# klemens-floege/oneprot

Hardware: AMD Instinct MI355X
Metric: protein-pairs/sec/node (seq+struct-token, L=512, ESM-2-150M) (higher is better)
Workload: dtype bf16; 1 GPU; cfg-2: seq<->struct_token sub-step, facebook/esm2_t30_150M_UR50D / facebook/esm2_t30_150M_UR50D, L=512, 256 pairs/GPU per modality, global batch 256, output_dim 1024, CLIP local_loss+gather_with_grad, L1 0.01, Adam 1e-3, clip 1.0, sequence encoder frozen (reference default), random-init weights; global_batch=256, seq_len=512, parallelism=dp1, frozen_sequence_encoder=True

## Files before the change

include/oneprot_hip.h:

```cpp
#ifndef ONEPROT_HIP_H
#define ONEPROT_HIP_H
#include <stddef.h>
#include <stdint.h>
#ifdef __cplusplus
extern "C" {
#endif

int oneprot_abi_version(void);

int oneprot_esm_embed_fwd(const int64_t* ids, const float* table, float* x, float* row_scale, int B, int L, int d, int vocab,
                          int pad_id, int mask_id, int token_dropout, void* stream);
size_t oneprot_esm_embed_bwd_workspace(int T, int d, int vocab);
int oneprot_esm_embed_bwd(const int64_t* ids, const float* dx, const float* row_scale, float* dtable, void* workspace, int B, int L, int d,
                          int vocab, int pad_id, int mask_id, int token_dropout, int accumulate, void* stream);
int oneprot_bert_embed_fwd(const int64_t* ids, const float* word, const float* pos, const float* type0, const float* gamma, const float* beta,
                           float* x_f32, void* x_bf16, int B, int L, int d, int vocab, float eps, void* stream);

int oneprot_layernorm_fwd(const void* x, int x_is_bf16, const float* gamma, const float* beta, void* y_bf16, float* y_f32, float* mean,
                          float* rstd, int64_t T, int d, float eps, void* stream);
size_t oneprot_layernorm_bwd_workspace(int d);
int oneprot_layernorm_bwd(const void* dy, int dy_mode, const float* wrow, int L, const void* x, int x_is_bf16, const float* gamma,
                          const float* mean, const float* rstd, const float* add_to, float* dx, void* dx_bf16 ,
                          float* dgamma, float* dbeta, void* workspace, int64_t T, int d, int accumulate_param_grads, void* stream);
int oneprot_lnpool_fwd(const float* x, const int64_t* ids, int pad_id, const float* gamma, const float* beta, float* pooled, float* mean,
// ... 52 lines not shown

int oneprot_attn_fwd(const void* q, const void* k, const void* v, const float* key_bias, void* ctx, float* lse, int B, int H, int L, int hd,
                     void* stream);
size_t oneprot_attn_bwd_workspace(int B, int H, int L);
int oneprot_attn_bwd(const void* q, const void* k, const void* v, const float* key_bias, const void* ctx, const void* dctx, const float* lse,
                     const float* rope_cos, const float* rope_sin, float q_scale, void* dqkv, void* workspace, int B, int H, int L, int hd,
                     void* stream);
int oneprot_attn_fwd_dropout(const void* q, const void* k, const void* v, const float* key_bias, void* ctx, float* lse, int B, int H, int L, int hd,
                             float p, uint64_t seed, uint64_t stream_id, void* stream);
int oneprot_attn_bwd_dropout(const void* q, const void* k, const void* v, const float* key_bias, const void* ctx, const void* dctx, const float* lse,
                             const float* rope_cos, const float* rope_sin, float q_scale, void* dqkv, void* workspace, int B, int H, int L, int hd,
                             float p, uint64_t seed, uint64_t stream_id, void* stream);
int oneprot_attn_dropout_keep(void* keep, int B, int H, int L, float p, uint64_t seed, uint64_t stream_id, void* stream);
void oneprot_attn_force_bwd_path(int path);
void oneprot_attn_force_fwd_path(int path);

int oneprot_gelu_f32(const float* x, float* y, int64_t n, void* stream);
int oneprot_gelu_bwd_f32(const float* x, const float* dy, float* dx, int64_t n, void* stream);
int oneprot_l2norm_fwd(const float* x, float* y, float* inv_norm, int R, int D, float scale, void* stream);
int oneprot_l2norm_bwd(const float* y, const float* dy, const float* inv_norm, float* dx, int R, int D, float scale, float l1_coef, void* stream);
int oneprot_ce_fwd_bwd(float* logits, float* loss_sum, float* row_loss_ws , int R, int C, int label_offset, float row_weight, void* stream);
int oneprot_siglip_fwd_bwd(float* logits, float* loss_sum, float* row_loss_ws , int B, float logit_bias, int negative_only, void* stream);
int oneprot_siglip_fwd_bwd_dev(float* logits, float* loss_sum, float* row_loss_ws , int B, const float* logit_bias_dev, int negative_only, void* stream);
int oneprot_diag_rank(const float* logits, int* rank_row, int* rank_col, int N, void* stream);
int oneprot_abs_sum(const float* x, float* out_sum, void* workspace , int64_t n, float coef, void* stream);

int oneprot_dot_f32(const float* x, const float* y, float* out_sum, void* workspace , int64_t n, float coef, void* stream);

int oneprot_l1_bwd(const float* x, float* dx, int64_t n, float coef, const float* upstream, int accumulate, void* stream);
int oneprot_scale_by_device_scalar(float* x, int64_t n, const float* s, void* stream);
// ... 48 lines not shown
```

oneprot_amd/csrc/attention.hip:

```cpp
#include "common.h"
#include "sched_ws.h"
#include "../../include/oneprot_hip.h"
#include <float.h>
#include <atomic>
void* dynamic_tiles_workspace();

#define LOG2E 1.4426950408889634f
#define KC 256
#define RESCALE_THR 10.0f

template <int HD> struct Cfg {
  static constexpr int HDP = HD < 32 ? 32 : HD;
  static constexpr int NCH = HDP / 8;
  static constexpr int KSTEPS = HD / 16;
  static constexpr int DBLK = HDP / 32;
  static constexpr int ROWB = HDP * 2;
};

template <int HDP> __device__ __forceinline__ int swz(int row, int chunk) {
  return HDP == 32 ? (chunk ^ ((row >> 2) & 3)) : (chunk ^ ((row >> 1) & 7));
}

template <int HD> struct TileRegs { u32x4 v[KC * Cfg<HD>::NCH / 256]; };
template <int HD>
// ... 405 lines not shown
    typedef Cfg<HD> C;
    const unsigned char* kt = sK + t * 32 * C::ROWB;
    const unsigned char* vt = sV + t * 32 * C::ROWB;
#pragma unroll
    for (int st = 0; st < C::KSTEPS; ++st) k[st] = *reinterpret_cast<const bf8_t*>(kt + fo.koff(st));
#pragma unroll
    for (int sb = 0; sb < 2; ++sb)
#pragma unroll
      for (int d = 0; d < C::DBLK; ++d) v[sb][d] = fo.vt(vt, sb, d);
  }
};

#ifndef FWD3_PRIO
#define FWD3_PRIO 3
#endif
template <int HD, int NB, bool BOOK, class Side>
__device__ __forceinline__ void fwd_tile_fast(const unsigned char* sK, const unsigned char* sV, const float* sBias, bool have_bias, int nkeys, int t,
                                              const bf8_t (&qf)[NB][Cfg<HD>::KSTEPS], RowState<HD> (&st)[NB], int lane, const FragOff<HD>& fo,
                                              const TileFrags<HD>& cur, TileFrags<HD>* nxt, int t_next, Side&& side) {
  typedef Cfg<HD> C;
  const int h = lane >> 5;
  const bf8_t (&kf)[C::KSTEPS] = cur.k;
  f32x16 s[NB];
#if FWD3_PRIO == 1 || FWD3_PRIO == 3
  __builtin_amdgcn_s_setprio(1);
#elif FWD3_PRIO == 2
  __builtin_amdgcn_s_setprio(0);
#endif
#ifdef FWD2_ABL_NOQK
#pragma unroll
  for (int b = 0; b < NB; ++b) { s[b] = zero16(); asm volatile("" : "+v"(s[b])); }
#else
  if constexpr (BOOK) {
    const bf8_t ke = key_entry(sBias, have_bias, nkeys, t, lane);
    u32x4 q1 = {0u, 0u, 0u, 0u};
    if (h == 0) q1.y = 0x3F800000u;
#pragma unroll
    for (int b = 0; b < NB; ++b) s[b] = MFMA32(ke, __builtin_bit_cast(bf8_t, q1), zero16());
#pragma unroll
    for (int k = 0; k < C::KSTEPS; ++k)
#pragma unroll
      for (int b = 0; b < NB; ++b) s[b] = MFMA32(kf[k], qf[b][k], s[b]);
  } else {
#pragma unroll
    for (int b = 0; b < NB; ++b) s[b] = MFMA32(kf[0], qf[b][0], zero16());
#pragma unroll
    for (int k = 1; k < C::KSTEPS; ++k)
#pragma unroll
// ... 65 lines not shown
      unsigned w01, w2;
      split3_bf16(-st.m, w01, w2);
      st.qe.x = w01; st.qe.y = w2 | 0x3F800000u;
    }
    st.first = false;
  }
#pragma unroll
  for (int e = 0; e < 16; ++e) s[e] = __builtin_amdgcn_exp2f(s[e]);
#pragma unroll
  for (int sb = 0; sb < 2; ++sb) {
    const bf8_t pf = pack8(s, sb);
    st.add_frag(pf);
#pragma unroll
    for (int d = 0; d < C::DBLK; ++d) st.acc[d] = MFMA32(rd_tr<HD>(sV, t * 32, sb, d, lane), pf, st.acc[d]);
  }
}

template <int HD, int NB, class Side>
__device__ __forceinline__ void fwd_chunk_fast(const unsigned char* sK, const unsigned char* sV, const float* sBias, bool have_bias, int nkeys, int nt,
                                               unsigned long long NZ, unsigned long long DEAD, const bf8_t (&qf)[NB][Cfg<HD>::KSTEPS], RowState<HD> (&st)[NB], int lane,
                                               Side&& side) {
  FragOff<HD> fo;
  fo.init(lane);
  unsigned long long special = (NZ | (NZ >> 1) | (NZ >> 2) | (NZ >> 3)) & 0x1111111111111111ull;
  if (nt < 16) special |= ~0ull << (4 * nt);
  int t = 0;
  while (t < nt) {
    const unsigned long long rest = special >> (4 * t);
    const int run_end = rest ? t + (__builtin_ctzll(rest) >> 2) : nt;
    if (t < run_end) {
      TileFrags<HD> fa, fb;
      fa.load(sK, sV, t, fo);
      for (; t + 1 < run_end; t += 2) {
        fwd_tile_fast<HD, NB, false>(sK, sV, sBias, have_bias, nkeys, t, qf, st, lane, fo, fa, &fb, t + 1, side);
        fwd_tile_fast<HD, NB, false>(sK, sV, sBias, have_bias, nkeys, t + 1, qf, st, lane, fo, fb, &fa, t + 2, side);
      }
      if (t < run_end) { fwd_tile_fast<HD, NB, false>(sK, sV, sBias, have_bias, nkeys, t, qf, st, lane, fo, fa, nullptr, 0, side); ++t; }
    }
    if (t < nt) {
      if (tile_class(NZ, DEAD, t) == 1) {
        TileFrags<HD> f;
        f.load(sK, sV, t, fo);
        fwd_tile_fast<HD, NB, true>(sK, sV, sBias, have_bias, nkeys, t, qf, st, lane, fo, f, nullptr, 0, side);
      }
      ++t;
// ... 219 lines not shown
  unsigned keep;
  asm volatile("s_mov_b32 %0, m0\n\ts_mov_b32 m0, %3\n\ts_nop 0\n\tglobal_load_lds_dwordx4 %1, %2\n\ts_mov_b32 m0, %0" : "=&s"(keep) : "v"(voff), "s"(sbase), "s"(lds_dst) : "memory");
}
__device__ __forceinline__ void glds4_s(unsigned voff, const void* sbase, unsigned lds_dst) {
  unsigned keep;
  asm volatile("s_mov_b32 %0, m0\n\ts_mov_b32 m0, %3\n\ts_nop 0\n\tglobal_load_lds_dword %1, %2\n\ts_mov_b32 m0, %0" : "=&s"(keep) : "v"(voff), "s"(sbase), "s"(lds_dst) : "memory");
}

struct Fwd3 {
  static constexpr int ROWS = 512;
  static constexpr int TILE = ROWS * 64;
  static constexpr int BUF = 2 * TILE + ROWS * 4;
  static constexpr int TOTAL = 2 * BUF;
};

template <int HD>
__global__ void __launch_bounds__(512, 2) k_attn_fwd3(const bf16_t* __restrict__ q, const bf16_t* __restrict__ k, const bf16_t* __restrict__ v,
                                                   const float* __restrict__ key_bias, bf16_t* __restrict__ ctx, float* __restrict__ lse_out, int B, int H,
                                                   int L, unsigned* __restrict__ sched) {
  typedef Cfg<HD> C;
  static_assert(C::ROWB == 64, "k_attn_fwd3 stages 64-byte rows");
  extern __shared__ __attribute__((aligned(16))) unsigned char smem[];
  const unsigned lds0 = (unsigned)(uintptr_t)LDS_PTR(smem);
  const int lane = threadIdx.x & 63, wave = __builtin_amdgcn_readfirstlane(threadIdx.x >> 6), h = lane >> 5, r = lane & 31;
  const int nw = blockDim.x >> 6;
  const int nbh = B * H, per_xcd = (nbh + 7) >> 3, nslot = gridDim.x >> 3;
  const int xcd = blockIdx.x & 7;
  const int bh_end = min(nbh, (xcd + 1) * per_xcd);
  unsigned* const relay = reinterpret_cast<unsigned*>(smem + Fwd3::TOTAL);
  int bh, bh_next;
  if (sched) {
    if (threadIdx.x == 0) {
      unsigned* head = sched + SW_HEAD(xcd);
      const unsigned t0 = sw_draw(head), t1 = sw_draw(head);
      relay[0] = t0 < 0x3fffffffu ? t0 : 0x3fffffffu; relay[1] = t1 < 0x3fffffffu ? t1 : 0x3fffffffu;
    }
    __syncthreads();
    bh = xcd * per_xcd + __builtin_amdgcn_readfirstlane((int)relay[0]);
    bh_next = xcd * per_xcd + __builtin_amdgcn_readfirstlane((int)relay[1]);
    __syncthreads();
  } else {
    bh = xcd * per_xcd + (int)(blockIdx.x >> 3);
    bh_next = bh + nslot;
  }
  const int q0 = wave * 64;
  const bool active = q0 < L;
  int qidx[2], qrow[2];
#pragma unroll
  for (int b = 0; b < 2; ++b) { qidx[b] = q0 + 32 * b + r; qrow[b] = qidx[b] < L ? qidx[b] : L - 1; }
  const int nrows = (L + 31) & ~31;
  const int npieces = nrows >> 4;
  const int dm = H * HD;
  const unsigned char* zero = reinterpret_cast<const unsigned char*>(g_attn_zero_page);

  const int my_pieces = npieces > wave ? (npieces - wave + nw - 1) / nw : 0;
  const int n_biasp = (nrows + 63) >> 6;
  const unsigned kv_lane_off = (unsigned)(lane >> 2) * (HD * 2) + (unsigned)((((lane & 3) ^ ((lane >> 4) & 3)) < HD / 8) ? ((lane & 3) ^ ((lane >> 4) & 3)) : 0) * 16u;
  auto dma_piece = [&](int item, int buf, int i) {
    const unsigned dst0 = lds0 + buf * Fwd3::BUF;
    if (i < 2 * my_pieces) {
      const int p = wave + nw * (i >> 1);
      const unsigned char* base = reinterpret_cast<const unsigned char*>(((i & 1) ? v : k) + (size_t)item * L * HD);
      const unsigned dst = dst0 + ((i & 1) ? Fwd3::TILE : 0) + p * 1024;
      if (16 * p + 16 <= L) glds16_s(kv_lane_off, base + (size_t)p * (16 * HD * 2), dst);
      else {
        const int row = 16 * p + (lane >> 2);
        const int ch = (lane & 3) ^ ((row >> 2) & 3);
        const bool ok = row < L && ch < HD / 8;
        glds16_addr(ok ? base + (size_t)row * (HD * 2) + ch * 16 : zero, dst);
      }
    } else {
      const float* br = key_bias + (size_t)(item / H) * L + 64 * wave;
      if (64 * wave + 64 <= L) glds4_s((unsigned)lane * 4u, br, dst0 + 2 * Fwd3::TILE + wave * 256);
      else glds4_addr(64 * wave + lane < L ? (const void*)(br + lane) : (const void*)zero, dst0 + 2 * Fwd3::TILE + wave * 256);
    }
  };
  const int n_dma = 2 * my_pieces + ((key_bias && wave < n_biasp) ? 1 : 0);
  constexpr int NQ = 2 * C::KSTEPS;
  constexpr int NST = 2 * (RowOut<HD>::NPIECE + 1);
  auto load_q1 = [&](int item, bf8_t (&dstq)[2][C::KSTEPS], int i) {
#pragma unroll
    for (int b = 0; b < 2; ++b)
#pragma unroll
      for (int st = 0; st < C::KSTEPS; ++st)
        if (i == b * C::KSTEPS + st) dstq[b][st] = *reinterpret_cast<const bf8_t*>(q + ((size_t)item * L + qrow[b]) * HD + 16 * st + 8 * h);
  };
  auto store1 = [&](const RowOut<HD> (&o)[2], int item, int i) {
#pragma unroll
    for (int b = 0; b < 2; ++b) {
      bf16_t* dst = ctx + ((size_t)(item / H) * L + qidx[b]) * dm + (item % H) * HD;
#pragma unroll
      for (int pc = 0; pc < RowOut<HD>::NPIECE; ++pc)
        if (i == b * (RowOut<HD>::NPIECE + 1) + pc && qidx[b] < L) o[b].store_piece(pc, dst, h);
      if (i == b * (RowOut<HD>::NPIECE + 1) + RowOut<HD>::NPIECE && lse_out && h == 0 && qidx[b] < L) lse_out[(size_t)item * L + qidx[b]] = o[b].lse;
    }
  };

  bf8_t qf[2][C::KSTEPS], qn[2][C::KSTEPS];
  if (bh < bh_end) {
    for (int i = 0; i < n_dma; ++i) dma_piece(bh, 0, i);
    for (int i = 0; i < NQ; ++i) load_q1(bh, qf, i);
  }
  RowOut<HD> pend[2];
  int pend_bh = -1, buf = 0;
  int slab_no = 0;
  unsigned drawn_v = 0;
  const unsigned relay_lds = lds0 + Fwd3::TOTAL;
  const int draw_lane = (sched != nullptr && wave == 0) ? 1 : 0;
  while (bh < bh_end) {
    FWD3_T(0);
    asm volatile("s_waitcnt vmcnt(0)" ::: "memory");
    FWD3_T(1);
    if (sched && slab_no > 0) {
      int late;
      const int t = draw_result(drawn_v, late);
      if (wave == 0) lds_write32(relay_lds + 4u * (slab_no & 1), (unsigned)(t < 0 || t > 0x3fffffff ? 0x3fffffff : t));
      asm volatile("s_waitcnt lgkmcnt(0)" ::: "memory");
    }
    __builtin_amdgcn_s_barrier();
    FWD3_T(2);
    if (sched && slab_no > 0) {
      const unsigned rv = lds_read32(relay_lds + 4u * (slab_no & 1));
      asm volatile("s_waitcnt lgkmcnt(0)" ::: "memory");
      bh_next = xcd * per_xcd + first_lane(rv);
    }
    drawn_v = draw_async(sched ? sched + SW_HEAD(xcd) : nullptr, draw_lane & (int)((unsigned)(bh_next - bh_end) >> 31));
#ifdef FWD3_DEPHASE
    if (wave >= 4) __builtin_amdgcn_s_sleep(FWD3_DEPHASE);
#endif
#pragma unroll
    for (int b = 0; b < 2; ++b)
#pragma unroll
      for (int st = 0; st < C::KSTEPS; ++st) asm volatile("" : "+v"(qf[b][st]));
    const int nxt = bh_next;
    const bool more = nxt < bh_end;
#ifndef FWD3_ABL_NOQ
    if (more)
      for (int i = 0; i < NQ; ++i) load_q1(nxt, qn, i);
#else
    for (int b = 0; b < 2; ++b) for (int st = 0; st < C::KSTEPS; ++st) qn[b][st] = qf[b][st];
#endif
    const int n_pairs = more ? my_pieces : 0;
    const bool bias_piece = more && key_bias && wave < n_biasp;
    const bool have_stores = pend_bh >= 0 && active;
    const int n_slots = n_pairs + 3;
    const unsigned char* const kbase = reinterpret_cast<const unsigned char*>(k + (size_t)nxt * L * HD);
    const unsigned char* const vbase = reinterpret_cast<const unsigned char*>(v + (size_t)nxt * L * HD);
    const unsigned dst_next = lds0 + (buf ^ 1) * Fwd3::BUF;
    int vm_i = 0;
    auto vm_step = [&]() {
      const int i = vm_i;
      if (i >= n_slots) return;
      vm_i = i + 1;
      if (i < n_pairs) {
#ifndef FWD3_ABL_NODMA
        const int p = wave + nw * i;
        const unsigned dk = dst_next + p * 1024;
        if (16 * p + 16 <= L) {
          glds16_s(kv_lane_off, kbase + (size_t)p * (16 * HD * 2), dk);
          glds16_s(kv_lane_off, vbase + (size_t)p * (16 * HD * 2), dk + Fwd3::TILE);
        } else {
          const int row = 16 * p + (lane >> 2);
          const int ch = (lane & 3) ^ ((row >> 2) & 3);
          const bool ok = row < L && ch < HD / 8;
          glds16_addr(ok ? kbase + (size_t)row * (HD * 2) + ch * 16 : zero, dk);
          glds16_addr(ok ? vbase + (size_t)row * (HD * 2) + ch * 16 : zero, dk + Fwd3::TILE);
        }
#endif
      } else if (i == n_pairs) {
#ifndef FWD3_ABL_NODMA
        if (bias_piece) {
          const float* br = key_bias + (size_t)(nxt / H) * L + 64 * wave;
          if (64 * wave + 64 <= L) glds4_s((unsigned)lane * 4u, br, dst_next + 2 * Fwd3::TILE + wave * 256);
          else glds4_addr(64 * wave + lane < L ? (const void*)(br + lane) : (const void*)zero, dst_next + 2 * Fwd3::TILE + wave * 256);
        }
#endif
      } else if (have_stores) {
#ifndef FWD3_ABL_NOSTORE
        if (i == n_pairs + 1) {
#pragma unroll
          for (int j = 0; j < NST / 2; ++j) store1(pend, pend_bh, j);
        } else {
#pragma unroll
          for (int j = NST / 2; j < NST; ++j) store1(pend, pend_bh, j);
        }
#endif
      }
    };
    const int e_all = n_slots;
    FWD3_T(3);
    if (active) {
      const unsigned char* sK = smem + buf * Fwd3::BUF;
      const unsigned char* sV = sK + Fwd3::TILE;
      const float* sBias = reinterpret_cast<const float*>(sK + 2 * Fwd3::TILE);
      const bool have_bias = key_bias != nullptr;
      unsigned long long NZ, DEAD;
      tile_class_masks(sBias, Fwd3::ROWS, L, have_bias, lane, NZ, DEAD);
      const int nt = nrows >> 5;
      RowState<HD> st[2];
      st[0].reset(h); st[1].reset(h);
      fwd_chunk_fast<HD, 2>(sK, sV, sBias, have_bias, L, nt, NZ, DEAD, qf, st, lane, [&] { vm_step(); });
      while (vm_i < e_all) vm_step();
      st[0].finish_sum(); st[1].finish_sum();
      FWD3_T(4);
#ifndef FWD2_NOFALLBACK
#pragma unroll
      for (int b = 0; b < 2; ++b)
        if (__any(!st[b].sums_ok())) {
          st[b].reset(h);
          fwd_chunk_exact<HD>(sK, sV, sBias, have_bias, L, nt, NZ, DEAD, qf[b], st[b], lane);
          st[b].finish_sum();
        }
#endif
      pend[0].from(st[0]); pend[1].from(st[1]);
    } else {
      while (vm_i < e_all) vm_step();
    }
    FWD3_T(5);
    ++slab_no;
    pend_bh = bh;
    bh = nxt; buf ^= 1;
    if (!sched) bh_next = bh + nslot;
#pragma unroll
    for (int b = 0; b < 2; ++b)
#pragma unroll
      for (int st = 0; st < C::KSTEPS; ++st) qf[b][st] = qn[b][st];
  }
  if (pend_bh >= 0 && active)
    for (int i = 0; i < NST; ++i) store1(pend, pend_bh, i);
  if (sched && threadIdx.x == 0) sw_leave(sched, gridDim.x, (unsigned)slab_no, (unsigned)nbh);
}

#define REDO_SLOTS 8
#define REDO_SLABS 32768
__device__ unsigned g_fwd3w_redo_any[REDO_SLOTS];
__device__ unsigned g_fwd3w_redo_slab[REDO_SLOTS * REDO_SLABS];
template <int HD> struct Fwd3W {
  static constexpr int CK = 256;
  static constexpr int TILE = CK * Cfg<HD>::ROWB;
  static constexpr int BUF = 2 * TILE + CK * 4;
  static constexpr int TOTAL = 2 * BUF + 4096;
};

template <int HD, int NB, bool BOOK, bool NEXT, class Side>
__device__ __forceinline__ void fwd_tile_fast_ip(const unsigned char* sK, const unsigned char* sV, const float* sBias, bool have_bias, int nkeys, int t,
// ... 190 lines not shown
          RowOut<HD> o;
          o.from(st[b]);
          if (qidx[b] < L) o.store(dst0 + (size_t)qidx[b] * dm, lse0 ? lse0 + qidx[b] : nullptr, h);
        }
      }
#pragma unroll
      for (int b = 0; b < 2; ++b)
#pragma unroll
        for (int s_ = 0; s_ < C::KSTEPS; ++s_) qf[b][s_] = qn[b][s_];
    }
    bh = nbh_; c = nc; buf ^= 1;
  }
}

static int g_attn_fwd_path = -1;
extern "C" void oneprot_attn_force_fwd_path(int path) { g_attn_fwd_path = path < 0 ? -1 : (path > 2 ? 1 : path); }

template <int HD>
static int launch_fwd2(const void* q, const void* k, const void* v, const float* key_bias, void* ctx, float* lse, int B, int H, int L, hipStream_t s) {
  static int ok = -1;
  if (ok < 0) ok = hipFuncSetAttribute((const void*)k_attn_fwd2<HD>, hipFuncAttributeMaxDynamicSharedMemorySize, Fwd2<HD>::TOTAL) == hipSuccess ? 1 : 0;
  if (!ok) { (void)hipGetLastError(); return OP_EINVAL; }
  const int nqb = (L + 255) / 256;
  const int nbh8 = ((B * H + 7) / 8) * 8;
  const int waves = L >= 256 ? 8 : (L + 31) / 32;
  hipLaunchKernelGGL(k_attn_fwd2<HD>, dim3(nbh8 * nqb), dim3(64 * waves), Fwd2<HD>::TOTAL, s, (const bf16_t*)q, (const bf16_t*)k, (const bf16_t*)v, key_bias,
                     (bf16_t*)ctx, lse, B, H, L, nqb);
  return launch_status();
}

template <int HD>
static int launch_fwd3(const void* q, const void* k, const void* v, const float* key_bias, void* ctx, float* lse, int B, int H, int L, hipStream_t s) {
  static int ok = -1, n_cu = 0;
  if (ok < 0) {
    ok = hipFuncSetAttribute((const void*)k_attn_fwd3<HD>, hipFuncAttributeMaxDynamicSharedMemorySize, Fwd3::TOTAL + 16) == hipSuccess ? 1 : 0;
    int dev = 0; hipDeviceProp_t prop;
    if (hipGetDevice(&dev) != hipSuccess || hipGetDeviceProperties(&prop, dev) != hipSuccess) ok = 0; else n_cu = prop.multiProcessorCount;
  }
  if (!ok) { (void)hipGetLastError(); return launch_fwd2<HD>(q, k, v, key_bias, ctx, lse, B, H, L, s); }
  const int waves = (L + 63) / 64;
  const int per_xcd = (B * H + 7) / 8;
  int nslot = n_cu / 8;
  if (nslot < 1) nslot = 1;
  if (nslot > per_xcd) nslot = per_xcd;
  hipLaunchKernelGGL(k_attn_fwd3<HD>, dim3(8 * nslot), dim3(64 * waves), Fwd3::TOTAL + 16, s, (const bf16_t*)q, (const bf16_t*)k, (const bf16_t*)v, key_bias,
                     (bf16_t*)ctx, lse, B, H, L, (unsigned*)dynamic_tiles_workspace());
  return launch_status();
}

template <int HD>
static int launch_fwd3w(const void* q, const void* k, const void* v, const float* key_bias, void* ctx, float* lse, int B, int H, int L, hipStream_t s) {
  static int ok = -1, n_cu = 0;
  if (ok < 0) {
    ok = hipFuncSetAttribute((const void*)k_attn_fwd3w<HD>, hipFuncAttributeMaxDynamicSharedMemorySize, Fwd3W<HD>::TOTAL) == hipSuccess ? 1 : 0;
    int dev = 0; hipDeviceProp_t prop;
    if (hipGetDevice(&dev) != hipSuccess || hipGetDeviceProperties(&prop, dev) != hipSuccess) ok = 0; else n_cu = prop.multiProcessorCount;
  }
  if (!ok) { (void)hipGetLastError(); return launch_fwd2<HD>(q, k, v, key_bias, ctx, lse, B, H, L, s); }
  const int waves = (L + 63) / 64;
  const int per_xcd = (B * H + 7) / 8;
  int nslot = n_cu / 8;
// ... 10 lines not shown
  hipLaunchKernelGGL(k_attn_fwd3w<HD>, dim3(8 * nslot), dim3(64 * waves), Fwd3W<HD>::TOTAL, s, (const bf16_t*)q, (const bf16_t*)k, (const bf16_t*)v, key_bias,
                     (bf16_t*)ctx, lse, B, H, L, any_w, slab_w, epoch);
  if (launch_status() != OP_OK) return OP_ELAUNCH;
  static int ok2 = -1;
  if (ok2 < 0) ok2 = hipFuncSetAttribute((const void*)k_attn_fwd2_redo<HD>, hipFuncAttributeMaxDynamicSharedMemorySize, Fwd2<HD>::TOTAL) == hipSuccess ? 1 : 0;
  if (!ok2) return OP_ELAUNCH;
  const int nqb = (L + 255) / 256;
  hipLaunchKernelGGL(k_attn_fwd2_redo<HD>, dim3(n_cu), dim3(512), Fwd2<HD>::TOTAL, s, (const bf16_t*)q, (const bf16_t*)k, (const bf16_t*)v, key_bias, (bf16_t*)ctx, lse,
                     B, H, L, nqb, (const unsigned*)any_w, (const unsigned*)slab_w, epoch);
  return launch_status();
}

template <int HD>
static int launch_fwd_nomax(const void* q, const void* k, const void* v, const float* key_bias, void* ctx, float* lse, int B, int H, int L, hipStream_t s) {
  if constexpr (HD <= 32) {
    if (L <= Fwd3::ROWS && g_attn_fwd_path != 2) return launch_fwd3<HD>(q, k, v, key_bias, ctx, lse, B, H, L, s);
  } else {
    if (L <= 512 && (long)B * H <= REDO_SLABS && g_attn_fwd_path != 2) return launch_fwd3w<HD>(q, k, v, key_bias, ctx, lse, B, H, L, s);
  }
  return launch_fwd2<HD>(q, k, v, key_bias, ctx, lse, B, H, L, s);
}

extern "C" int oneprot_attn_fwd(const void* q, const void* k, const void* v, const float* key_bias, void* ctx, float* lse, int B, int H, int L, int hd,
                                void* stream) {
  if (!q || !k || !v || !ctx || B <= 0 || H <= 0 || L <= 0) return OP_EINVAL;
  hipStream_t s = (hipStream_t)stream;
  if (g_attn_fwd_path != 0) {
    switch (hd) {
      case 16: return launch_fwd_nomax<16>(q, k, v, key_bias, ctx, lse, B, H, L, s);
      case 32: return launch_fwd_nomax<32>(q, k, v, key_bias, ctx, lse, B, H, L, s);
      case 64: return launch_fwd_nomax<64>(q, k, v, key_bias, ctx, lse, B, H, L, s);
      default: return OP_EINVAL;
    }
  }
  switch (hd) {
    case 16: return launch_fwd<16>(q, k, v, key_bias, ctx, lse, B, H, L, s);
    case 32: return launch_fwd<32>(q, k, v, key_bias, ctx, lse, B, H, L, s);
    case 64: return launch_fwd<64>(q, k, v, key_bias, ctx, lse, B, H, L, s);
    default: return OP_EINVAL;
  }
}

extern "C" int oneprot_attn_fwd_dropout(const void* q, const void* k, const void* v, const float* key_bias, void* ctx, float* lse, int B, int H, int L, int hd, float p,
                                        uint64_t seed, uint64_t stream_id, void* stream) {
  AttnDrop dr;
  if (!q || !k || !v || !ctx || B <= 0 || H <= 0 || L <= 0 || attn_drop_make(p, seed, stream_id, dr) != OP_OK) return OP_EINVAL;
  hipStream_t s = (hipStream_t)stream;
  switch (hd) {
    case 16: return launch_fwd_dropout<16>(q, k, v, key_bias, ctx, lse, B, H, L, dr, s);
    case 32: return launch_fwd_dropout<32>(q, k, v, key_bias, ctx, lse, B, H, L, dr, s);
    case 64: return launch_fwd_dropout<64>(q, k, v, key_bias, ctx, lse, B, H, L, dr, s);
    default: return OP_EINVAL;
  }
}

// ... 1226 lines not shown
```

oneprot_amd/hip.py:

```python
import ctypes
import os
from ctypes import c_float, c_int, c_int64, c_size_t, c_void_p

import torch

_HERE = os.path.dirname(os.path.abspath(__file__))
LIB_PATH = os.environ.get("ONEPROT_HIP_LIB") or os.path.join(_HERE, "liboneprot_hip.so")

ABI_VERSION = 7
EPI_BF16, EPI_F32, EPI_BIAS_GELU, EPI_BIAS_RESID, EPI_QKV_ROPE, EPI_GELU_BWD = range(6)
LOG2E = 1.4426950408889634


class HipLibraryMissing(RuntimeError):
    pass


class HipKernelError(RuntimeError):
    pass


P, I, L64, F, SZ = c_void_p, c_int, c_int64, c_float, c_size_t
U64 = ctypes.c_uint64

# ... 34 lines not shown
    "oneprot_gemm_force_shape": (None, [I]),
    "oneprot_gemm_tune": (None, [I, I]),
    "oneprot_gemm_bf16_tn_workspace": (SZ, [I, I]),
    "oneprot_gemm_tn_variant": (None, [I]),
    "oneprot_cu_reserve": (None, [I]),
    "oneprot_gemm_bf16_tn": (I, [P, P, L64, I, I, I, I, P, P, P, SZ, I, P]),
    "oneprot_sgemm": (I, [P, P, P, I, I, I, I, I, F, I, P]),
    "oneprot_attn_fwd": (I, [P, P, P, P, P, P, I, I, I, I, P]),
    "oneprot_attn_fwd_dropout": (I, [P, P, P, P, P, P, I, I, I, I, F, U64, U64, P]),
    "oneprot_attn_dropout_keep": (I, [P, I, I, I, F, U64, U64, P]),
    "oneprot_attn_bwd_dropout": (I, [P, P, P, P, P, P, P, P, P, F, P, P, I, I, I, I, F, U64, U64, P]),
    "oneprot_attn_bwd_workspace": (SZ, [I, I, I]),
    "oneprot_attn_bwd": (I, [P, P, P, P, P, P, P, P, P, F, P, P, I, I, I, I, P]),
    "oneprot_attn_force_bwd_path": (None, [I]),
    "oneprot_attn_force_fwd_path": (None, [I]),
    "oneprot_gelu_f32": (I, [P, P, L64, P]),
    "oneprot_gelu_bwd_f32": (I, [P, P, P, L64, P]),
    "oneprot_l2norm_fwd": (I, [P, P, P, I, I, F, P]),
    "oneprot_l2norm_bwd": (I, [P, P, P, P, I, I, F, F, P]),
    "oneprot_ce_fwd_bwd": (I, [P, P, P, I, I, I, F, P]),
    "oneprot_siglip_fwd_bwd": (I, [P, P, P, I, F, I, P]),
    "oneprot_siglip_fwd_bwd_dev": (I, [P, P, P, I, P, I, P]),
    "oneprot_diag_rank": (I, [P, P, P, I, P]),
    "oneprot_abs_sum": (I, [P, P, P, L64, F, P]),
    "oneprot_dot_f32": (I, [P, P, P, P, L64, F, P]),
    "oneprot_l1_bwd": (I, [P, P, L64, F, P, I, P]),
    "oneprot_scale_by_device_scalar": (I, [P, L64, P, P]),
    "oneprot_dropout_bf16": (I, [P, P, L64, F, U64, U64, P]),
    "oneprot_dropout_bwd_add_bf16": (I, [P, P, L64, F, U64, U64, P]),
    "oneprot_dropout_bwd_add_f32": (I, [P, P, L64, F, U64, U64, P]),
# ... 216 lines not shown
```

Baseline: 1182 protein-pairs/sec/node.

## Add four-query-block-per-wave attention forward kernel with software-pipelined QK/PV MFMAs

Adds k_attn_fwd4, a variant of the 64-row fwd3 attention forward in which each wave handles four 32-row query blocks instead of two. It uses a hand-scheduled pipeline that interleaves the PV MFMAs of the previous block, the QK MFMAs of the next block and the exp/pack work of the current block, with inline-asm MFMAs and explicit s_nop hazard padding. It is made the default for L>256 when no dynamic tile scheduler is in use. The goal is to hide MFMA latency and increase per-wave reuse of K/V fragments. In exchange it runs at lower occupancy (256 threads, one block) with static scheduling and relies on hand-counted wait states, which a new checker script verifies.

```diff
diff --git a/include/oneprot_hip.h b/include/oneprot_hip.h
--- a/include/oneprot_hip.h
+++ b/include/oneprot_hip.h
@@ -90,6 +90,7 @@
 int oneprot_attn_dropout_keep(void* keep, int B, int H, int L, float p, uint64_t seed, uint64_t stream_id, void* stream);
 void oneprot_attn_force_bwd_path(int path);
 void oneprot_attn_force_fwd_path(int path);
+int oneprot_attn_fwd_form(int hd, int L);
 
 int oneprot_gelu_f32(const float* x, float* y, int64_t n, void* stream);
 int oneprot_gelu_bwd_f32(const float* x, const float* dy, float* dx, int64_t n, void* stream);
diff --git a/oneprot_amd/csrc/attention.hip b/oneprot_amd/csrc/attention.hip
--- a/oneprot_amd/csrc/attention.hip
+++ b/oneprot_amd/csrc/attention.hip
@@ -443,6 +443,17 @@
 #ifndef FWD3_PRIO
 #define FWD3_PRIO 3
 #endif
+__device__ __forceinline__ f32x16 mfma32_sv_first(const bf8_t& a, const bf8_t& b, bool last) {
+  f32x16 d;
+  if (last) asm("s_nop 1\n\tv_mfma_f32_32x32x16_bf16 %0, %1, %2, 0\n\ts_nop 11" : "=&v"(d) : "v"(a), "v"(b));
+  else asm("s_nop 1\n\tv_mfma_f32_32x32x16_bf16 %0, %1, %2, 0" : "=&v"(d) : "v"(a), "v"(b));
+  return d;
+}
+__device__ __forceinline__ void mfma32_sv_acc(f32x16& c, const bf8_t& a, const bf8_t& b, bool last) {
+  if (last) asm("s_nop 1\n\tv_mfma_f32_32x32x16_bf16 %0, %1, %2, %0\n\ts_nop 11" : "+v"(c) : "v"(a), "v"(b));
+  else asm("s_nop 1\n\tv_mfma_f32_32x32x16_bf16 %0, %1, %2, %0" : "+v"(c) : "v"(a), "v"(b));
+}
+
 template <int HD, int NB, bool BOOK, class Side>
 __device__ __forceinline__ void fwd_tile_fast(const unsigned char* sK, const unsigned char* sV, const float* sBias, bool have_bias, int nkeys, int t,
                                               const bf8_t (&qf)[NB][Cfg<HD>::KSTEPS], RowState<HD> (&st)[NB], int lane, const FragOff<HD>& fo,
@@ -460,7 +471,26 @@
 #pragma unroll
   for (int b = 0; b < NB; ++b) { s[b] = zero16(); asm volatile("" : "+v"(s[b])); }
 #else
-  if constexpr (BOOK) {
+  if constexpr (NB == 4) {
+    if constexpr (BOOK) {
+      const bf8_t ke = key_entry(sBias, have_bias, nkeys, t, lane);
+      u32x4 q1 = {0u, 0u, 0u, 0u};
+      if (h == 0) q1.y = 0x3F800000u;
+#pragma unroll
+      for (int b = 0; b < NB; ++b) s[b] = mfma32_sv_first(ke, __builtin_bit_cast(bf8_t, q1), true);
+#pragma unroll
+      for (int k = 0; k < C::KSTEPS; ++k)
+#pragma unroll
+        for (int b = 0; b < NB; ++b) mfma32_sv_acc(s[b], kf[k], qf[b][k], k == C::KSTEPS - 1);
+    } else {
+#pragma unroll
+      for (int b = 0; b < NB; ++b) s[b] = mfma32_sv_first(kf[0], qf[b][0], C::KSTEPS == 1);
+#pragma unroll
+      for (int k = 1; k < C::KSTEPS; ++k)
+#pragma unroll
+        for (int b = 0; b < NB; ++b) mfma32_sv_acc(s[b], kf[k], qf[b][k], k == C::KSTEPS - 1);
+    }
+  } else if constexpr (BOOK) {
     const bf8_t ke = key_entry(sBias, have_bias, nkeys, t, lane);
     u32x4 q1 = {0u, 0u, 0u, 0u};
     if (h == 0) q1.y = 0x3F800000u;
@@ -556,6 +586,89 @@
 #pragma unroll
     for (int d = 0; d < C::DBLK; ++d) st.acc[d] = MFMA32(rd_tr<HD>(sV, t * 32, sb, d, lane), pf, st.acc[d]);
   }
+}
+
+template <int HD> struct Frag4 {
+  bf8_t k[Cfg<HD>::KSTEPS];
+  bf8_t v[2][Cfg<HD>::DBLK];
+  __device__ __forceinline__ void load_k(const unsigned char* sK, int t, const FragOff<HD>& fo) {
+    const unsigned char* kt = sK + t * 32 * Cfg<HD>::ROWB;
+#pragma unroll
+    for (int st = 0; st < Cfg<HD>::KSTEPS; ++st) k[st] = *reinterpret_cast<const bf8_t*>(kt + fo.koff(st));
+  }
+  __device__ __forceinline__ void load_v(const unsigned char* sV, int t, const FragOff<HD>& fo) {
+    const unsigned char* vt = sV + t * 32 * Cfg<HD>::ROWB;
+#pragma unroll
+    for (int sb = 0; sb < 2; ++sb)
+#pragma unroll
+      for (int d = 0; d < Cfg<HD>::DBLK; ++d) v[sb][d] = fo.vt(vt, sb, d);
+  }
+};
+
+template <int HD, bool FIRST, class Side>
+__device__ __forceinline__ void fwd4_tile(const unsigned char* sK, const unsigned char* sV, int t, const bf8_t (&qf)[4][Cfg<HD>::KSTEPS], RowState<HD> (&st)[4],
+                                          f32x16 (&s)[4], bf8_t (&pf)[2], Frag4<HD>& fr, const FragOff<HD>& fo, Side&& side) {
+  typedef Cfg<HD> C;
+  side();
+#pragma unroll
+  for (int b = 0; b < 4; ++b) {
+    const int pb = (b + 3) & 3, nb = (b + 2) & 3;
+    const bool do_pv = !(FIRST && b == 0);
+    bf8_t pn[2];
+#pragma unroll
+    for (int g = 0; g < 4; ++g) {
+      __builtin_amdgcn_sched_barrier(0);
+      if (g < 2) {
+        if (do_pv) {
+#pragma unroll
+          for (int d = 0; d < C::DBLK; ++d) st[pb].acc[d] = MFMA32(fr.v[g][d], pf[g], st[pb].acc[d]);
+        }
+      } else if (g - 2 < C::KSTEPS) {
+        if (g == 2) s[nb] = mfma32_sv_first(fr.k[0], qf[nb][0], false);
+        else mfma32_sv_acc(s[nb], fr.k[g - 2], qf[nb][g - 2], false);
+      }
+      if (b == 0 && g == 2) fr.load_v(sV, t, fo);
+      __builtin_amdgcn_sched_barrier(0);
+      if (g < 2) {
+#pragma unroll
+        for (int e = 8 * g; e < 8 * g + 8; ++e) s[b][e] = __builtin_amdgcn_exp2f(s[b][e]);
+      } else {
+        pn[g - 2] = pack8(s[b], g - 2);
+        st[b].add_frag(pn[g - 2]);
+      }
+    }
+    if (C::KSTEPS > 2) {
+#pragma unroll
+      for (int k = 2; k < C::KSTEPS; ++k) mfma32_sv_acc(s[nb], fr.k[k], qf[nb][k], false);
+    }
+    if (b == 1) fr.load_k(sK, t + 1, fo);
+    __builtin_amdgcn_sched_barrier(0);
+    pf[0] = pn[0]; pf[1] = pn[1];
+  }
+  asm volatile("s_nop 3");
+}
+
+template <int HD, class Side>
+__device__ __forceinline__ void fwd4_run(const unsigned char* sK, const unsigned char* sV, int t, int run_end, const bf8_t (&qf)[4][Cfg<HD>::KSTEPS],
+                                         RowState<HD> (&st)[4], const FragOff<HD>& fo, Side&& side) {
+  typedef Cfg<HD> C;
+  Frag4<HD> fr;
+  f32x16 s[4];
+  bf8_t pf[2];
+  fr.load_k(sK, t, fo);
+#pragma unroll
+  for (int b = 0; b < 2; ++b) {
+    s[b] = mfma32_sv_first(fr.k[0], qf[b][0], false);
+#pragma unroll
+    for (int k = 1; k < C::KSTEPS; ++k) mfma32_sv_acc(s[b], fr.k[k], qf[b][k], false);
+  }
+  asm volatile("s_nop 11" : "+v"(s[0]), "+v"(s[1]));
+  fwd4_tile<HD, true>(sK, sV, t, qf, st, s, pf, fr, fo, side);
+  for (++t; t < run_end; ++t) fwd4_tile<HD, false>(sK, sV, t, qf, st, s, pf, fr, fo, side);
+#pragma unroll
+  for (int g = 0; g < 2; ++g)
+#pragma unroll
+    for (int d = 0; d < C::DBLK; ++d) st[3].acc[d] = MFMA32(fr.v[g][d], pf[g], st[3].acc[d]);
 }
 
 template <int HD, int NB, class Side>
@@ -570,7 +683,9 @@
   while (t < nt) {
     const unsigned long long rest = special >> (4 * t);
     const int run_end = rest ? t + (__builtin_ctzll(rest) >> 2) : nt;
-    if (t < run_end) {
+    if constexpr (NB == 4) {
+      if (t < run_end) { fwd4_run<HD>(sK, sV, t, run_end, qf, st, fo, side); t = run_end; }
+    } else if (t < run_end) {
       TileFrags<HD> fa, fb;
       fa.load(sK, sV, t, fo);
       for (; t + 1 < run_end; t += 2) {
@@ -820,17 +935,19 @@
   static constexpr int TOTAL = 2 * BUF;
 };
 
-template <int HD>
-__global__ void __launch_bounds__(512, 2) k_attn_fwd3(const bf16_t* __restrict__ q, const bf16_t* __restrict__ k, const bf16_t* __restrict__ v,
-                                                   const float* __restrict__ key_bias, bf16_t* __restrict__ ctx, float* __restrict__ lse_out, int B, int H,
-                                                   int L, unsigned* __restrict__ sched) {
+template <int HD, int NB, bool DYN>
+__device__ __forceinline__ void fwd3_body(const bf16_t* __restrict__ q, const bf16_t* __restrict__ k, const bf16_t* __restrict__ v,
+                                          const float* __restrict__ key_bias, bf16_t* __restrict__ ctx, float* __restrict__ lse_out, int B, int H, int L,
+                                          unsigned* __restrict__ sched_arg, const unsigned nthreads, const unsigned nblocks) {
   typedef Cfg<HD> C;
-  static_assert(C::ROWB == 64, "k_attn_fwd3 stages 64-byte rows");
+  static_assert(C::ROWB == 64, "k_attn_fwd3 / k_attn_fwd4 stage 64-byte rows");
+  static_assert(NB == 2 || NB == 4, "two or four query blocks per wave");
+  unsigned* const sched = DYN ? sched_arg : nullptr;
   extern __shared__ __attribute__((aligned(16))) unsigned char smem[];
   const unsigned lds0 = (unsigned)(uintptr_t)LDS_PTR(smem);
   const int lane = threadIdx.x & 63, wave = __builtin_amdgcn_readfirstlane(threadIdx.x >> 6), h = lane >> 5, r = lane & 31;
-  const int nw = blockDim.x >> 6;
-  const int nbh = B * H, per_xcd = (nbh + 7) >> 3, nslot = gridDim.x >> 3;
+  const int nw = nthreads >> 6;
+  const int nbh = B * H, per_xcd = (nbh + 7) >> 3, nslot = nblocks >> 3;
   const int xcd = blockIdx.x & 7;
   const int bh_end = min(nbh, (xcd + 1) * per_xcd);
   unsigned* const relay = reinterpret_cast<unsigned*>(smem + Fwd3::TOTAL);
@@ -849,11 +966,11 @@
     bh = xcd * per_xcd + (int)(blockIdx.x >> 3);
     bh_next = bh + nslot;
   }
-  const int q0 = wave * 64;
+  const int q0 = wave * (32 * NB);
   const bool active = q0 < L;
-  int qidx[2], qrow[2];
-#pragma unroll
-  for (int b = 0; b < 2; ++b) { qidx[b] = q0 + 32 * b + r; qrow[b] = qidx[b] < L ? qidx[b] : L - 1; }
+  int qidx[NB], qrow[NB];
+#pragma unroll
+  for (int b = 0; b < NB; ++b) { qidx[b] = q0 + 32 * b + r; qrow[b] = qidx[b] < L ? qidx[b] : L - 1; }
   const int nrows = (L + 31) & ~31;
   const int npieces = nrows >> 4;
   const int dm = H * HD;
@@ -862,6 +979,14 @@
   const int my_pieces = npieces > wave ? (npieces - wave + nw - 1) / nw : 0;
   const int n_biasp = (nrows + 63) >> 6;
   const unsigned kv_lane_off = (unsigned)(lane >> 2) * (HD * 2) + (unsigned)((((lane & 3) ^ ((lane >> 4) & 3)) < HD / 8) ? ((lane & 3) ^ ((lane >> 4) & 3)) : 0) * 16u;
+  constexpr int BPW = NB / 2;
+  const int my_biasp = key_bias ? min(max(n_biasp - BPW * wave, 0), BPW) : 0;
+  auto bias_piece_dma = [&](int item, unsigned dst0, int j) {
+    const int bp = BPW * wave + j;
+    const float* br = key_bias + (size_t)(item / H) * L + 64 * bp;
+    if (64 * bp + 64 <= L) glds4_s((unsigned)lane * 4u, br, dst0 + 2 * Fwd3::TILE + bp * 256);
+    else glds4_addr(64 * bp + lane < L ? (const void*)(br + lane) : (const void*)zero, dst0 + 2 * Fwd3::TILE + bp * 256);
+  };
   auto dma_piece = [&](int item, int buf, int i) {
     const unsigned dst0 = lds0 + buf * Fwd3::BUF;
     if (i < 2 * my_pieces) {
@@ -876,38 +1001,37 @@
         glds16_addr(ok ? base + (size_t)row * (HD * 2) + ch * 16 : zero, dst);
       }
     } else {
-      const float* br = key_bias + (size_t)(item / H) * L + 64 * wave;
-      if (64 * wave + 64 <= L) glds4_s((unsigned)lane * 4u, br, dst0 + 2 * Fwd3::TILE + wave * 256);
-      else glds4_addr(64 * wave + lane < L ? (const void*)(br + lane) : (const void*)zero, dst0 + 2 * Fwd3::TILE + wave * 256);
+      bias_piece_dma(item, dst0, i - 2 * my_pieces);
     }
   };
-  const int n_dma = 2 * my_pieces + ((key_bias && wave < n_biasp) ? 1 : 0);
-  constexpr int NQ = 2 * C::KSTEPS;
-  constexpr int NST = 2 * (RowOut<HD>::NPIECE + 1);
-  auto load_q1 = [&](int item, bf8_t (&dstq)[2][C::KSTEPS], int i) {
-#pragma unroll
-    for (int b = 0; b < 2; ++b)
+  const int n_dma = 2 * my_pieces + my_biasp;
+  constexpr int NQ = NB * C::KSTEPS;
+  constexpr int NSTB = RowOut<HD>::NPIECE + 1;
+  constexpr int NST = NB * NSTB;
+  auto load_q1 = [&](int item, bf8_t (&dstq)[NB][C::KSTEPS], int i) {
+#pragma unroll
+    for (int b = 0; b < NB; ++b)
 #pragma unroll
       for (int st = 0; st < C::KSTEPS; ++st)
         if (i == b * C::KSTEPS + st) dstq[b][st] = *reinterpret_cast<const bf8_t*>(q + ((size_t)item * L + qrow[b]) * HD + 16 * st + 8 * h);
   };
-  auto store1 = [&](const RowOut<HD> (&o)[2], int item, int i) {
-#pragma unroll
-    for (int b = 0; b < 2; ++b) {
+  auto store1 = [&](const RowOut<HD> (&o)[NB], int item, int i) {
+#pragma unroll
+    for (int b = 0; b < NB; ++b) {
       bf16_t* dst = ctx + ((size_t)(item / H) * L + qidx[b]) * dm + (item % H) * HD;
 #pragma unroll
       for (int pc = 0; pc < RowOut<HD>::NPIECE; ++pc)
-        if (i == b * (RowOut<HD>::NPIECE + 1) + pc && qidx[b] < L) o[b].store_piece(pc, dst, h);
-      if (i == b * (RowOut<HD>::NPIECE + 1) + RowOut<HD>::NPIECE && lse_out && h == 0 && qidx[b] < L) lse_out[(size_t)item * L + qidx[b]] = o[b].lse;
+        if (i == b * NSTB + pc && qidx[b] < L) o[b].store_piece(pc, dst, h);
+      if (i == b * NSTB + RowOut<HD>::NPIECE && lse_out && h == 0 && qidx[b] < L) lse_out[(size_t)item * L + qidx[b]] = o[b].lse;
     }
   };
 
-  bf8_t qf[2][C::KSTEPS], qn[2][C::KSTEPS];
+  bf8_t qf[NB][C::KSTEPS], qn[NB][C::KSTEPS];
   if (bh < bh_end) {
     for (int i = 0; i < n_dma; ++i) dma_piece(bh, 0, i);
     for (int i = 0; i < NQ; ++i) load_q1(bh, qf, i);
   }
-  RowOut<HD> pend[2];
+  RowOut<HD> pend[NB];
   int pend_bh = -1, buf = 0;
   int slab_no = 0;
   unsigned drawn_v = 0;
@@ -930,12 +1054,13 @@
       asm volatile("s_waitcnt lgkmcnt(0)" ::: "memory");
       bh_next = xcd * per_xcd + first_lane(rv);
     }
-    drawn_v = draw_async(sched ? sched + SW_HEAD(xcd) : nullptr, draw_lane & (int)((unsigned)(bh_next - bh_end) >> 31));
+    if constexpr (DYN)
+      drawn_v = draw_async(sched ? sched + SW_HEAD(xcd) : nullptr, draw_lane & (int)((unsigned)(bh_next - bh_end) >> 31));
 #ifdef FWD3_DEPHASE
-    if (wave >= 4) __builtin_amdgcn_s_sleep(FWD3_DEPHASE);
+    if (NB == 2 && wave >= 4) __builtin_amdgcn_s_sleep(FWD3_DEPHASE);
 #endif
 #pragma unroll
-    for (int b = 0; b < 2; ++b)
+    for (int b = 0; b < NB; ++b)
 #pragma unroll
       for (int st = 0; st < C::KSTEPS; ++st) asm volatile("" : "+v"(qf[b][st]));
     const int nxt = bh_next;
@@ -944,12 +1069,12 @@
     if (more)
       for (int i = 0; i < NQ; ++i) load_q1(nxt, qn, i);
 #else
-    for (int b = 0; b < 2; ++b) for (int st = 0; st < C::KSTEPS; ++st) qn[b][st] = qf[b][st];
+    for (int b = 0; b < NB; ++b) for (int st = 0; st < C::KSTEPS; ++st) qn[b][st] = qf[b][st];
 #endif
     const int n_pairs = more ? my_pieces : 0;
-    const bool bias_piece = more && key_bias && wave < n_biasp;
+    const int n_biasp_next = more ? my_biasp : 0;
     const bool have_stores = pend_bh >= 0 && active;
-    const int n_slots = n_pairs + 3;
+    const int n_slots = n_pairs + 1 + NB;
     const unsigned char* const kbase = reinterpret_cast<const unsigned char*>(k + (size_t)nxt * L * HD);
     const unsigned char* const vbase = reinterpret_cast<const unsigned char*>(v + (size_t)nxt * L * HD);
     const unsigned dst_next = lds0 + (buf ^ 1) * Fwd3::BUF;
@@ -975,21 +1100,19 @@
 #endif
       } else if (i == n_pairs) {
 #ifndef FWD3_ABL_NODMA
-        if (bias_piece) {
-          const float* br = key_bias + (size_t)(nxt / H) * L + 64 * wave;
-          if (64 * wave + 64 <= L) glds4_s((unsigned)lane * 4u, br, dst_next + 2 * Fwd3::TILE + wave * 256);
-          else glds4_addr(64 * wave + lane < L ? (const void*)(br + lane) : (const void*)zero, dst_next + 2 * Fwd3::TILE + wave * 256);
-        }
+#pragma unroll
+        for (int j = 0; j < BPW; ++j)
+          if (j < n_biasp_next) bias_piece_dma(nxt, dst_next, j);
 #endif
       } else if (have_stores) {
 #ifndef FWD3_ABL_NOSTORE
-        if (i == n_pairs + 1) {
-#pragma unroll
-          for (int j = 0; j < NST / 2; ++j) store1(pend, pend_bh, j);
-        } else {
-#pragma unroll
-          for (int j = NST / 2; j < NST; ++j) store1(pend, pend_bh, j);
-        }
+#pragma unroll
+        for (int b = 0; b < NB; ++b)
+          if (b == NB - 1 || i == n_pairs + 1 + b) {
+#pragma unroll
+            for (int j = 0; j < NSTB; ++j) store1(pend, pend_bh, b * NSTB + j);
+            break;
+          }
 #endif
       }
     };
@@ -1003,22 +1126,25 @@
       unsigned long long NZ, DEAD;
       tile_class_masks(sBias, Fwd3::ROWS, L, have_bias, lane, NZ, DEAD);
       const int nt = nrows >> 5;
-      RowState<HD> st[2];
-      st[0].reset(h); st[1].reset(h);
-      fwd_chunk_fast<HD, 2>(sK, sV, sBias, have_bias, L, nt, NZ, DEAD, qf, st, lane, [&] { vm_step(); });
+      RowState<HD> st[NB];
+#pragma unroll
+      for (int b = 0; b < NB; ++b) st[b].reset(h);
+      fwd_chunk_fast<HD, NB>(sK, sV, sBias, have_bias, L, nt, NZ, DEAD, qf, st, lane, [&] { vm_step(); });
       while (vm_i < e_all) vm_step();
-      st[0].finish_sum(); st[1].finish_sum();
+#pragma unroll
+      for (int b = 0; b < NB; ++b) st[b].finish_sum();
       FWD3_T(4);
 #ifndef FWD2_NOFALLBACK
 #pragma unroll
-      for (int b = 0; b < 2; ++b)
+      for (int b = 0; b < NB; ++b)
         if (__any(!st[b].sums_ok())) {
           st[b].reset(h);
           fwd_chunk_exact<HD>(sK, sV, sBias, have_bias, L, nt, NZ, DEAD, qf[b], st[b], lane);
           st[b].finish_sum();
         }
 #endif
-      pend[0].from(st[0]); pend[1].from(st[1]);
+#pragma unroll
+      for (int b = 0; b < NB; ++b) pend[b].from(st[b]);
     } else {
       while (vm_i < e_all) vm_step();
     }
@@ -1028,13 +1154,27 @@
     bh = nxt; buf ^= 1;
     if (!sched) bh_next = bh + nslot;
 #pragma unroll
-    for (int b = 0; b < 2; ++b)
+    for (int b = 0; b < NB; ++b)
 #pragma unroll
       for (int st = 0; st < C::KSTEPS; ++st) qf[b][st] = qn[b][st];
   }
   if (pend_bh >= 0 && active)
     for (int i = 0; i < NST; ++i) store1(pend, pend_bh, i);
-  if (sched && threadIdx.x == 0) sw_leave(sched, gridDim.x, (unsigned)slab_no, (unsigned)nbh);
+  if (sched && threadIdx.x == 0) sw_leave(sched, nblocks, (unsigned)slab_no, (unsigned)nbh);
+}
+
+template <int HD>
+__global__ void __launch_bounds__(512, 2) k_attn_fwd3(const bf16_t* __restrict__ q, const bf16_t* __restrict__ k, const bf16_t* __restrict__ v,
+                                                   const float* __restrict__ key_bias, bf16_t* __restrict__ ctx, float* __restrict__ lse_out, int B, int H,
+                                                   int L, unsigned* __restrict__ sched) {
+  fwd3_body<HD, 2, true>(q, k, v, key_bias, ctx, lse_out, B, H, L, sched, blockDim.x, gridDim.x);
+}
+
+template <int HD>
+__global__ void __launch_bounds__(256, 1) k_attn_fwd4(const bf16_t* __restrict__ q, const bf16_t* __restrict__ k, const bf16_t* __restrict__ v,
+                                                   const float* __restrict__ key_bias, bf16_t* __restrict__ ctx, float* __restrict__ lse_out, int B, int H,
+                                                   int L) {
+  fwd3_body<HD, 4, false>(q, k, v, key_bias, ctx, lse_out, B, H, L, nullptr, blockDim.x, gridDim.x);
 }
 
 #define REDO_SLOTS 8
@@ -1255,7 +1395,15 @@
 }
 
 static int g_attn_fwd_path = -1;
-extern "C" void oneprot_attn_force_fwd_path(int path) { g_attn_fwd_path = path < 0 ? -1 : (path > 2 ? 1 : path); }
+extern "C" void oneprot_attn_force_fwd_path(int path) { g_attn_fwd_path = path < 0 ? -1 : (path > 4 ? 1 : path); }
+#ifndef FWD4_DEFAULT
+#define FWD4_DEFAULT 1
+#endif
+static int fwd_rows64_form(int L) {
+  if (dynamic_tiles_workspace() != nullptr || g_attn_fwd_path == 3) return 3;
+  if (g_attn_fwd_path == 4) return 4;
+  return FWD4_DEFAULT && L > 256 ? 4 : 3;
+}
 
 template <int HD>
 static int launch_fwd2(const void* q, const void* k, const void* v, const float* key_bias, void* ctx, float* lse, int B, int H, int L, hipStream_t s) {
@@ -1286,6 +1434,25 @@
   if (nslot > per_xcd) nslot = per_xcd;
   hipLaunchKernelGGL(k_attn_fwd3<HD>, dim3(8 * nslot), dim3(64 * waves), Fwd3::TOTAL + 16, s, (const bf16_t*)q, (const bf16_t*)k, (const bf16_t*)v, key_bias,
                      (bf16_t*)ctx, lse, B, H, L, (unsigned*)dynamic_tiles_workspace());
+  return launch_status();
+}
+
+template <int HD>
+static int launch_fwd4(const void* q, const void* k, const void* v, const float* key_bias, void* ctx, float* lse, int B, int H, int L, hipStream_t s) {
+  static int ok = -1, n_cu = 0;
+  if (ok < 0) {
+    ok = hipFuncSetAttribute((const void*)k_attn_fwd4<HD>, hipFuncAttributeMaxDynamicSharedMemorySize, Fwd3::TOTAL + 16) == hipSuccess ? 1 : 0;
+    int dev = 0; hipDeviceProp_t prop;
+    if (hipGetDevice(&dev) != hipSuccess || hipGetDeviceProperties(&prop, dev) != hipSuccess) ok = 0; else n_cu = prop.multiProcessorCount;
+  }
+  if (!ok) { (void)hipGetLastError(); return launch_fwd2<HD>(q, k, v, key_bias, ctx, lse, B, H, L, s); }
+  const int waves = (L + 127) / 128;
+  const int per_xcd = (B * H + 7) / 8;
+  int nslot = n_cu / 8;
+  if (nslot < 1) nslot = 1;
+  if (nslot > per_xcd) nslot = per_xcd;
+  hipLaunchKernelGGL(k_attn_fwd4<HD>, dim3(8 * nslot), dim3(64 * waves), Fwd3::TOTAL + 16, s, (const bf16_t*)q, (const bf16_t*)k, (const bf16_t*)v, key_bias,
+                     (bf16_t*)ctx, lse, B, H, L);
   return launch_status();
 }
 
@@ -1326,7 +1493,8 @@
 template <int HD>
 static int launch_fwd_nomax(const void* q, const void* k, const void* v, const float* key_bias, void* ctx, float* lse, int B, int H, int L, hipStream_t s) {
   if constexpr (HD <= 32) {
-    if (L <= Fwd3::ROWS && g_attn_fwd_path != 2) return launch_fwd3<HD>(q, k, v, key_bias, ctx, lse, B, H, L, s);
+    if (L <= Fwd3::ROWS && g_attn_fwd_path != 2)
+      return fwd_rows64_form(L) == 4 ? launch_fwd4<HD>(q, k, v, key_bias, ctx, lse, B, H, L, s) : launch_fwd3<HD>(q, k, v, key_bias, ctx, lse, B, H, L, s);
   } else {
     if (L <= 512 && (long)B * H <= REDO_SLABS && g_attn_fwd_path != 2) return launch_fwd3w<HD>(q, k, v, key_bias, ctx, lse, B, H, L, s);
   }
@@ -1351,6 +1519,12 @@
     case 64: return launch_fwd<64>(q, k, v, key_bias, ctx, lse, B, H, L, s);
     default: return OP_EINVAL;
   }
+}
+
+extern "C" int oneprot_attn_fwd_form(int hd, int L) {
+  if (g_attn_fwd_path == 0 || (hd != 16 && hd != 32 && hd != 64)) return 0;
+  if (g_attn_fwd_path == 2 || L > 512) return 2;
+  return hd <= 32 ? fwd_rows64_form(L) : 3;
 }
 
 extern "C" int oneprot_attn_fwd_dropout(const void* q, const void* k, const void* v, const float* key_bias, void* ctx, float* lse, int B, int H, int L, int hd, float p,
diff --git a/oneprot_amd/csrc/check_mfma_vgpr.py b/oneprot_amd/csrc/check_mfma_vgpr.py
--- /dev/null
+++ b/oneprot_amd/csrc/check_mfma_vgpr.py
@@ -0,0 +1,75 @@
+#!/usr/bin/env python3
+import re
+import sys
+
+STATES = 12
+
+
+def regs_of(tok):
+    out = set()
+    for m in re.finditer(r"\bv\[(\d+):(\d+)\]", tok):
+        out.update(range(int(m.group(1)), int(m.group(2)) + 1))
+    for m in re.finditer(r"\bv(\d+)\b", tok):
+        out.add(int(m.group(1)))
+    return out
+
+
+def check(name, lines):
+    errs = []
+    code = []
+    for l in lines:
+        t = l.split(";")[0].strip()
+        if not t or t.startswith("."):
+            if t.startswith(".LBB") and t.endswith(":"):
+                code.append(t)
+            continue
+        code.append(t)
+    n = 0
+    for i, t in enumerate(code):
+        m = re.match(r"v_mfma_\w+ (v\[\d+:\d+\]), ([^,]+), ([^,]+), (.+)$", t)
+        if not m:
+            continue
+        n += 1
+        dst = regs_of(m.group(1))
+        states = 0
+        for u in code[i + 1:]:
+            if states >= STATES:
+                break
+            if u.endswith(":") or u.startswith("s_cbranch") or u.startswith("s_branch") or u.startswith("s_endpgm"):
+                errs.append(f"{name}: `{t}` is followed by `{u}` after {states} wait states")
+                break
+            mn = re.match(r"s_nop (\d+)", u)
+            if mn:
+                states += int(mn.group(1)) + 1
+                continue
+            if regs_of(u) & dst:
+                mm = re.match(r"v_mfma_\w+ (v\[\d+:\d+\]), ([^,]+), ([^,]+), (v\[\d+:\d+\])$", u)
+                if mm and mm.group(1) == m.group(1) and mm.group(4) == m.group(1) and not (regs_of(mm.group(2)) | regs_of(mm.group(3))) & dst:
+                    break
+                errs.append(f"{name}: `{u}` touches the result of `{t}` after {states} wait states")
+                break
+            states += 1
+    return n, errs
+
+
+def main(paths):
+    bad = total = kernels = 0
+    for path in paths:
+        s = open(path).read()
+        for m in re.finditer(r"^(_Z11k_attn_fwd4ILi\d+E\w+):[^\n]*\n", s, re.M):
+            end = s.index(".Lfunc_end", m.end())
+            n, errs = check(m.group(1), s[m.end():end].split("\n"))
+            kernels += 1
+            total += n
+            for e in errs:
+                print("MFMA-VGPR:", e)
+            bad += len(errs)
+    if kernels == 0 or total == 0:
+        print("MFMA-VGPR: no k_attn_fwd4 kernel with VGPR-destination MFMAs found in", paths)
+        return 1
+    print(f"check_mfma_vgpr: {kernels} kernels, {total} MFMAs with VGPR destinations, {bad} violations")
+    return 1 if bad else 0
+
+
+if __name__ == "__main__":
+    sys.exit(main(sys.argv[1:]))
diff --git a/oneprot_amd/hip.py b/oneprot_amd/hip.py
--- a/oneprot_amd/hip.py
+++ b/oneprot_amd/hip.py
@@ -72,6 +72,7 @@
     "oneprot_attn_bwd": (I, [P, P, P, P, P, P, P, P, P, F, P, P, I, I, I, I, P]),
     "oneprot_attn_force_bwd_path": (None, [I]),
     "oneprot_attn_force_fwd_path": (None, [I]),
+    "oneprot_attn_fwd_form": (I, [I, I]),
     "oneprot_gelu_f32": (I, [P, P, L64, P]),
     "oneprot_gelu_bwd_f32": (I, [P, P, P, L64, P]),
     "oneprot_l2norm_fwd": (I, [P, P, P, I, I, F, P]),
```

Measured after the change: 1157 protein-pairs/sec/node. 2.1% lower.
